# urw7rs/diffusion-models-made-easy

Hardware: AMD Instinct MI355X
Metric: denoising steps/sec + training images/sec, DDPM UNet CIFAR10 32×32 @1/2/4/8 GPU (higher is better)
Workload: dtype bf16

## Files before the change

### diffusion-models-made-easy_amd/csrc/conv_common.h

```cpp
#pragma once
#include <stdlib.h>

#include "common.h"

namespace dmme {

typedef float f32x16 __attribute__((ext_vector_type(16)));
typedef float f32x4 __attribute__((ext_vector_type(4)));
typedef __bf16 bf16x8 __attribute__((ext_vector_type(8)));
typedef f16 f16x8 __attribute__((ext_vector_type(8)));
template <typename T>
struct Vec8 {
    typedef T type __attribute__((ext_vector_type(8)));
};
template <typename T>
__device__ __forceinline__ void unpack8(const uint4& raw, float (&v)[8]) {
    const typename Vec8<T>::type x = __builtin_bit_cast(typename Vec8<T>::type, raw);
#pragma unroll
    for (int e = 0; e < 8; ++e) v[e] = (float)x[e];
}
template <typename T>
__device__ __forceinline__ uint4 pack8(const float (&v)[8]) {
    typename Vec8<T>::type x;
#pragma unroll
    for (int e = 0; e < 8; ++e) x[e] = (T)v[e];
    return __builtin_bit_cast(uint4, x);
}

constexpr int ROW_DATA = 128;
constexpr int ROW_PITCH = ROW_DATA + 16;

__device__ __forceinline__ int swz_off(int row, int chunk) { return row * ROW_DATA + ((chunk ^ ((row >> 1) & 7)) << 4); }

typedef __attribute__((address_space(3))) char lds_c;
__device__ __forceinline__ void glds16(const void* gsrc, unsigned lds_byte_addr) {
#if defined(__HIP_DEVICE_COMPILE__)
    __builtin_amdgcn_global_load_lds(gsrc, (lds_c*)(size_t)lds_byte_addr, 16, 0, 0);
#else
    (void)gsrc;
    (void)lds_byte_addr;
#endif
}
__device__ __forceinline__ void glds16_hidden(const void* gsrc, unsigned lds_byte_addr) {
#if defined(__HIP_DEVICE_COMPILE__)
    asm volatile("s_mov_b32 m0, %1\n\ts_nop 0\n\tglobal_load_lds_dwordx4 %0, off" ::"v"(gsrc), "s"(lds_byte_addr) : "m0");
#else
    (void)gsrc;
    (void)lds_byte_addr;
#endif
}
__device__ __forceinline__ void glds16_hidden_s(const void* sbase, unsigned lane_off, unsigned lds_byte_addr) {
#if defined(__HIP_DEVICE_COMPILE__)
    asm volatile("s_mov_b32 m0, %2\n\ts_nop 0\n\tglobal_load_lds_dwordx4 %0, %1" ::"v"(lane_off), "s"(sbase), "s"(lds_byte_addr) : "m0");
#else
    (void)sbase;
    (void)lane_off;
    (void)lds_byte_addr;
#endif
}
__device__ __forceinline__ void wait_vm_all() {
#if defined(__HIP_DEVICE_COMPILE__)
    asm volatile("s_waitcnt vmcnt(0)" ::: "memory");
#endif
}
__device__ __forceinline__ void wait_lgkm_all() {
#if defined(__HIP_DEVICE_COMPILE__)
    asm volatile("s_waitcnt lgkmcnt(0)" ::: "memory");
#endif
}
__device__ __forceinline__ void lds_barrier() {
#if defined(__HIP_DEVICE_COMPILE__)
    asm volatile("s_waitcnt lgkmcnt(0)" ::: "memory");
    __builtin_amdgcn_s_barrier();
    asm volatile("" ::: "memory");
#endif
}
template <int N>
__device__ __forceinline__ void wait_vm_keep() {
#if defined(__HIP_DEVICE_COMPILE__)
    asm volatile("s_waitcnt vmcnt(%0)" ::"n"(N) : "memory");
    asm volatile("s_waitcnt lgkmcnt(0)" ::: "memory");
#endif
}

template <typename T>
struct Frag;
template <>
struct Frag<float> {
    static constexpr int KC = 32;
    static constexpr int EPV = 4;
};
template <>
struct Frag<bf16> {
    static constexpr int KC = 64;
    static constexpr int EPV = 8;
};
template <>
struct Frag<f16> {
    static constexpr int KC = 64;
    static constexpr int EPV = 8;
};

__device__ __forceinline__ void mma_group(const uint4& a, const uint4& b, f32x16& acc, float*) {
    const f32x4 av = __builtin_bit_cast(f32x4, a), bv = __builtin_bit_cast(f32x4, b);
#pragma unroll
    for (int j = 0; j < 4; ++j) acc = __builtin_amdgcn_mfma_f32_32x32x2f32(av[j], bv[j], acc, 0, 0, 0);
}
__device__ __forceinline__ void mma_group(const uint4& a, const uint4& b, f32x16& acc, bf16*) {
    acc = __builtin_amdgcn_mfma_f32_32x32x16_bf16(__builtin_bit_cast(bf16x8, a), __builtin_bit_cast(bf16x8, b), acc, 0, 0, 0);
}
__device__ __forceinline__ void mma_group(const uint4& a, const uint4& b, f32x16& acc, f16*) {
    acc = __builtin_amdgcn_mfma_f32_32x32x16_f16(__builtin_bit_cast(f16x8, a), __builtin_bit_cast(f16x8, b), acc, 0, 0, 0);
}
template <typename T>
__device__ __forceinline__ void mma16(const uint4& a, const uint4& b, f32x16& acc) {
    mma_group(a, b, acc, (T*)nullptr);
}
template <typename T, typename A, typename B>
__device__ __forceinline__ f32x16 mma16v(const A& a, const B& b, f32x16 acc) {
    mma_group(__builtin_bit_cast(uint4, a), __builtin_bit_cast(uint4, b), acc, (T*)nullptr);
    return acc;
}

struct X3 {};
template <typename T, bool ACC3>
struct MmaTag {
    typedef T type;
};
template <>
struct MmaTag<float, true> {
    typedef X3 type;
};
typedef float f32x2 __attribute__((ext_vector_type(2)));
typedef __bf16 bf16x2 __attribute__((ext_vector_type(2)));
__device__ __forceinline__ float fma_plain(float a, float b, float c) {
    float d;
    asm("v_fma_f32 %0, %1, %2, %3" : "=v"(d) : "v"(a), "v"(b), "v"(c));
    return d;
}
__device__ __forceinline__ float mul_plain(float a, float b) {
    float d;
    asm("v_mul_f32 %0, %1, %2" : "=v"(d) : "v"(a), "v"(b));
    return d;
}
__device__ __forceinline__ float add_plain(float a, float b) {
    float d;
    asm("v_add_f32 %0, %1, %2" : "=v"(d) : "v"(a), "v"(b));
    return d;
}
__device__ __forceinline__ float sub_plain(float a, float b) {
    float d;
    asm("v_sub_f32 %0, %1, %2" : "=v"(d) : "v"(a), "v"(b));
    return d;
}
__device__ __forceinline__ float add1_plain(float a) {
    float d;
    asm("v_add_f32 %0, 1.0, %1" : "=v"(d) : "v"(a));
    return d;
}
__device__ __forceinline__ void pro_pair_plain(float x0, float x1, const f32x2& S, const f32x2& H, const f32x2& S2, const f32x2& H2, float& y0, float& y1) {
    float e0, e1;
    asm("v_fma_f32 %0, %4, %6, %8\n\t"
        "v_fma_f32 %2, %4, %10, %12\n\t"
        "v_fma_f32 %1, %5, %7, %9\n\t"
        "v_fma_f32 %3, %5, %11, %13\n\t"
        "v_exp_f32 %2, %2\n\t"
        "v_exp_f32 %3, %3\n\t"
        "v_add_f32 %2, 1.0, %2\n\t"
        "v_add_f32 %3, 1.0, %3\n\t"
        "v_rcp_f32 %2, %2\n\t"
        "v_rcp_f32 %3, %3\n\t"
        "v_mul_f32 %0, %0, %2\n\t"
        "v_mul_f32 %1, %1, %3"
        : "=&v"(y0), "=&v"(y1), "=&v"(e0), "=&v"(e1)
        : "v"(x0), "v"(x1), "v"(S[0]), "v"(S[1]), "v"(H[0]), "v"(H[1]), "v"(S2[0]), "v"(S2[1]), "v"(H2[0]), "v"(H2[1]));
}
typedef short s16x4 __attribute__((ext_vector_type(4)));
struct Split4 {
    uint2 hi, lo;
};
__device__ __forceinline__ unsigned pack_bf16(float a, float b) {
    const f32x2 v = {a, b};
    return __builtin_bit_cast(unsigned, __builtin_convertvector(v, bf16x2));
}
__device__ __forceinline__ Split4 split4(const uint4& v) {
    const f32x4 x = __builtin_bit_cast(f32x4, v);
    Split4 s;
    const unsigned h01 = pack_bf16(x[0], x[1]), h23 = pack_bf16(x[2], x[3]);
    s.hi = make_uint2(h01, h23);
    s.lo = make_uint2(pack_bf16(x[0] - __uint_as_float(h01 << 16), x[1] - __uint_as_float(h01 & 0xffff0000u)),
                      pack_bf16(x[2] - __uint_as_float(h23 << 16), x[3] - __uint_as_float(h23 & 0xffff0000u)));
    return s;
}
__device__ __forceinline__ void mma_x3(const Split4& a, const Split4& b, f32x16& acc) {
    const s16x4 ah = __builtin_bit_cast(s16x4, a.hi), al = __builtin_bit_cast(s16x4, a.lo);
// ... 746 lines not shown
```

### diffusion-models-made-easy_amd/csrc/conv_pipe.hip

```cpp
#include <stdio.h>

#include "conv_common.h"

namespace dmme {



template <typename T, int BM, int BN, int GT, int PIPE_UA, bool ACC3 = false>
__global__ void __launch_bounds__(256, GT == 9 ? 1 : 2) conv3x3_pipe_kernel(ConvArgs a, ConvTile g, int shTW, int shTH, int ksplit) {
    constexpr int KC = Frag<T>::KC, EPV = Frag<T>::EPV;
    constexpr int MI = BM / 64, NI = BN / 64;
    constexpr int UB = BN / 32;
    extern __shared__ __attribute__((aligned(16))) char lds[];
#define PIPE_STAMP(K) do { if (a.stamps && blockIdx.x < 2 && blockIdx.y == 0 && threadIdx.x == 0) a.stamps[blockIdx.x * 8 + (K)] = (long long)wall_clock64(); } while (0)
    PIPE_STAMP(0);
    char* ldsA = lds;
    char* ldsB = lds + (size_t)g.a_rows * ROW_DATA;
    constexpr bool DMAB_OK = sizeof(T) == 2 && GT == 3 && BN == 64;
    constexpr int B_BYTES = GT * BN * ROW_DATA;
    const bool dmab = DMAB_OK && a.dma_b;
    int cur = 0;
    float* gni_par = reinterpret_cast<float*>(ldsB + (size_t)B_BYTES * (dmab ? 2 : 1));

    const int tid = threadIdx.x, lane = tid & 63, wave = tid >> 6;
// ... 239 lines not shown
        }
        PIPE_STAMP(4);
        return;
    }
    if constexpr (BM == 64) {
        if (a.n_gno > 0) {
            const bool add_trow = a.tproj && a.nt != 1 && g.TN > 1;
            conv_epilogue_stage<T, BN, MI, NI>(a, acc, co0, wn0, r, h, wm0, n0, reinterpret_cast<float*>(lds), !add_trow);
            __syncthreads();
            conv_epilogue_store_direct<T, BN>(a, co0, n0, a.Hout * a.Wout, pix_of, reinterpret_cast<float*>(lds), add_trow);
            PIPE_STAMP(4);
            return;
        }
    }
    conv_epilogue<T, BM, BN, MI, NI>(a, acc, co0, wn0, r, h, wm0, n0, g.TN, pix_of, reinterpret_cast<float*>(lds), ty_blk * g.tiles_x + tx_blk);
    PIPE_STAMP(4);
#undef PIPE_STAMP
}

template <typename T>
__global__ void __launch_bounds__(256) conv_splitk_finish_kernel(ConvArgs a, int ksplit, int64_t total4) {
    const int C4 = a.Cout / 4, hw = a.Hout * a.Wout;
    const int64_t slice = (int64_t)a.N * hw * a.Cout;
    for (int64_t q = blockIdx.x * (int64_t)blockDim.x + threadIdx.x; q < total4; q += (int64_t)gridDim.x * blockDim.x) {
        const int64_t p = q / C4;
        const int c = (int)(q - p * C4) * 4;
        float4 v = *reinterpret_cast<const float4*>(a.splitk + p * a.Cout + c);
        for (int z = 1; z < ksplit; ++z) {
            const float4 u = *reinterpret_cast<const float4*>(a.splitk + z * slice + p * a.Cout + c);
            v.x += u.x; v.y += u.y; v.z += u.z; v.w += u.w;
        }
        float f[4] = {v.x, v.y, v.z, v.w};
        const int n = (int)(p / hw);
#pragma unroll
        for (int j = 0; j < 4; ++j) {
            float fold = a.bias ? a.bias[c + j] : 0.f;
            if (a.tproj) fold += a.tproj[(int64_t)(a.nt == 1 ? 0 : n) * a.tproj_ld + c + j];
            f[j] += fold;
            if (a.res1) f[j] += to_f(((const T*)a.res1)[p * a.Cout + c + j]);
            ((T*)a.dst)[p * a.Cout + c + j] = from_f<T>(f[j]);
        }
    }
}
static int pipe_ksplit(const ConvArgs& a, const ConvTile& g, int pick, int KC) {
    if (a.has_gni) return 1;
    const bool off = (debug_route("no_splitk") != 0);
    if (off || !a.splitk || pick != 3 || a.stride != 1 || a.gn_part || a.n_gno || a.out_silu || a.out_nchw || a.res2 || a.Cout % 4) return 1;
    const int64_t wgs = (int64_t)g.tiles_m * g.tiles_n;
    if (wgs > 128) return 1;
    int ks = (a.C1 + a.C2) / KC;
    const int room = (int)(256 / wgs);
    if (ks > room) ks = room;
    if (ks > 4) ks = 4;
    const int64_t out = (int64_t)a.N * a.Hout * a.Wout * a.Cout;
    while (ks > 1 && ks * out > a.splitk_cap) --ks;
    return ks < 1 ? 1 : ks;
}

#ifndef WS_CDMA
#define WS_CDMA 1
#endif
#ifndef WS_HYB
#define WS_HYB 0
#endif
#ifndef WS_SCHED2
#define WS_SCHED2 1
#endif
#ifndef WS_TP_UNROLL
#define WS_TP_UNROLL 9
#endif
template <typename T, int BN, int MI, int NI>
__device__ __forceinline__ void ws_stage16(const f32x16 (&acc)[MI][NI], T* row) {
    typedef T tx2 __attribute__((ext_vector_type(2)));
#pragma unroll
    for (int mi = 0; mi < MI; ++mi)
#pragma unroll
        for (int ni = 0; ni < NI; ++ni)
#pragma unroll
            for (int q = 0; q < 4; ++q) {
                const tx2 lo = {(T)acc[mi][ni][4 * q], (T)acc[mi][ni][4 * q + 1]}, hi = {(T)acc[mi][ni][4 * q + 2], (T)acc[mi][ni][4 * q + 3]};
                *reinterpret_cast<uint2*>(row + mi * 64 * (BN + kStage16Pad) + 32 * ni + 8 * q) = make_uint2(__builtin_bit_cast(unsigned, lo), __builtin_bit_cast(unsigned, hi));
            }
}
struct WsTile { int n0, oy0, ox0, co0, ts; };
__device__ __forceinline__ WsTile ws_tile_of(const ConvTile& g, int shTW, int shTH, int kt, int bn) {
    const int t = (int)blockIdx.x + kt * (int)gridDim.x;
    const int tile_n = t % g.tiles_n, tile_m = t / g.tiles_n;
    const int tiles_img = g.tiles_x * g.tiles_y;
    WsTile r;
    const int sp = tile_m % tiles_img;
    r.n0 = tile_m / tiles_img;
    r.oy0 = (sp / g.tiles_x) << shTH;
    r.ox0 = (sp % g.tiles_x) << shTW;
    r.co0 = tile_n * bn;
    r.ts = sp;
    return r;
}

__host__ __device__ inline int ws2_stage_pad(int a_bytes) { return a_bytes + 2 * 128 * ROW_DATA >= 64 * 1024 ? 0 : 64 * 1024 - 2 * 128 * ROW_DATA - a_bytes; }

__device__ __forceinline__ void ws_fill_par_gni(const ConvArgs& a, int n, bool writer, float* par, int Cin, int tid, int nthr) {
    for (int c = tid; c < Cin; c += nthr) {
        float sc, sh;
        const float dmk = a.dmask ? a.dmask[n * Cin + c] : 1.f;
        gn_in_scale_shift(a, n, c, Cin, writer, sc, sh);
        par[c] = sc * dmk;
        par[Cin + c] = sh * dmk;
        par[2 * Cin + c] = a.pro_silu ? -1.4426950408889634f * sc : 0.f;
        par[3 * Cin + c] = a.pro_silu ? -1.4426950408889634f * sh : -126.f;
    }
}

template <typename T, int SPLIT>
struct WsSplit {
    typedef T ts;
};
template <typename T>
struct WsSplit<T, 1> {
    typedef float ts;
};
template <typename T>
struct WsSplit<T, 2> {
    typedef float ts;
};
template <int PIPE_UA, typename T = bf16, int BM = 256, int SPLIT = 0, bool RSEG = false, bool E16 = false>
__global__ void __launch_bounds__(512, 1) conv3x3_ws2_kernel(ConvArgs a, ConvTile g, int shTW, int shTH, int ntiles) {
    constexpr int KC = 64, EPV = 8, BN = 128, MI = BM / 64, NI = 2, UB = BN / 32;
    constexpr bool CDMA = WS_CDMA != 0;
    constexpr bool SCHED2 = WS_SCHED2 != 0 && CDMA && SPLIT == 0;
    static_assert(!(SCHED2 && WS_HYB != 0), "the hybrid tap ownership counts the halo loads of the two-unit schedule");
    static_assert(!E16 || (SPLIT == 0 && BM == 256 && sizeof(T) == 2), "16-bit staging: 16-bit tensors, 256-pixel tiles");
    static_assert(!RSEG || (SPLIT == 0 && sizeof(T) == 2), "residual segment: 16-bit tensors");
    constexpr int KCR = SPLIT ? 32 : KC;
    constexpr int EPR = SPLIT ? 4 : EPV;
    typedef typename WsSplit<T, SPLIT>::ts TS;
    static_assert(SPLIT == 0 || (BM == 256 && dtype_of<T>::value == DMME_F16), "split passes: fp16 hi / lo on the 256-pixel tile");
    constexpr int R_BYTES = BN * ROW_DATA;
    constexpr int A_PITCH = ROW_DATA + 16;
    static_assert((BM == 256 && PIPE_UA == 11) || (BM == 128 && PIPE_UA == 7), "unit schedules below: 11 units over 9 stages, or 7 units over the first 7");
    typedef unsigned u32x4 __attribute__((ext_vector_type(4)));
    extern __shared__ __attribute__((aligned(16))) char lds[];
    const int a_bytes = g.a_rows * A_PITCH;
    const int Cin = a.C1 + a.C2;
    const int offA1 = a_bytes + 3 * R_BYTES, offR = a_bytes;
    float* par_base = reinterpret_cast<float*>(lds + 2 * a_bytes + 3 * R_BYTES + ws2_stage_pad(a_bytes));
    float* fold_base = par_base + 2 * 4 * Cin;
#define WS_FILL_FOLD(KT)                                                                              \
    if constexpr (E16) {                                                                              \
        if (tid < BN) {                                                                               \
            const TileXY ff_ = WS_TILE(KT);                                                           \
            const int co_ = ff_.co0 + tid;                                                            \
            float f_ = 0.f;                                                                           \
            if (co_ < a.Cout) {                                                                       \
                f_ = a.bias ? a.bias[co_] : 0.f;                                                      \
                if (a.r_bias) f_ += a.r_bias[co_];                                                    \
                if (a.tproj) f_ += a.tproj[(a.nt == 1 ? 0 : ff_.n0) * a.tproj_ld + co_];              \
            }                                                                                         \
            fold_base[((KT) & 1) * BN + tid] = f_;                                                    \
        }                                                                                             \
    }
#define WS_BUFA(p) (lds + (((p) & 1) ? offA1 : 0))
#define WS_RING(slot) (lds + offR + (slot) * R_BYTES)
#define WS_PAR(kt) (par_base + ((kt) & 1) * 4 * Cin)
#define WS_TILE(kt) ws_tile_of(g, shTW, shTH, (kt), BN)
    typedef WsTile TileXY;
    const int tid = threadIdx.x, lane = tid & 63, wave = tid >> 6;
    const bool producer = wave >= 4;
    const int nchunks = Cin / KCR;
    const int CinW = SPLIT ? 2 * Cin : Cin;
    const int Cres = RSEG ? a.r_C1 + a.r_C2 : 0;
    const int HS = Cres / 32;
    constexpr int RSL = 5;
    const int RT = HS + ((RSEG && (HS - 1) % RSL < 2) ? 1 : 0);
#define WS_RSA(k) ((k) < 2 ? lds + (k) * (BM * 64) : (k) == 2 ? lds + offR + 2 * R_BYTES : lds + offA1 + ((k) - 3) * (BM * 64))
#define WS_RSW(k) ((k) < 4 ? lds + offR + (k) * 8192 : lds + offA1 + 2 * (BM * 64))
    const int K = (ntiles - (int)blockIdx.x + (int)gridDim.x - 1) / (int)gridDim.x;
    const bool has_pro = a.scale || a.pro_silu || a.dmask;
#define WS_FILL_PAR_N(KT, NTHR)                                           \
    {                                                                     \
        float* par = WS_PAR(KT);                                          \
        const TileXY ft_ = WS_TILE(KT);                                   \
        if (a.has_gni) {                                                  \
            ws_fill_par_gni(a, ft_.n0, ft_.ts == 0 && ft_.co0 == 0, par, Cin, tid, NTHR); \
        } else {                                                          \
            const int pn0 = ft_.n0;                                       \
            for (int c = tid; c < Cin; c += (NTHR)) {                     \
                const int so = pn0 * Cin + c;                             \
                const float sc_ = a.scale ? a.scale[so] : 1.f, sh_ = a.scale ? a.shift[so] : 0.f, dm_ = a.dmask ? a.dmask[so] : 1.f; \
                par[c] = sc_ * dm_;                                       \
                par[Cin + c] = sh_ * dm_;                                 \
                par[2 * Cin + c] = a.pro_silu ? -1.4426950408889634f * sc_ : 0.f;    \
                par[3 * Cin + c] = a.pro_silu ? -1.4426950408889634f * sh_ : -126.f; \
            }                                                             \
        }                                                                 \
    }
#define WS_FILL_PAR(KT) WS_FILL_PAR_N(KT, 512)
    const int mTW = (1 << shTW) - 1, mTH = (1 << shTH) - 1;
    float gn_carry[2] = {0.f, 0.f};
    const bool estamp = tid == 0 && blockIdx.x == 0;
    int e_i = 0;
#define WS_ESTAMP() { if (estamp && a.stamps && e_i < 24) a.stamps[64 + e_i++] = (long long)clock64(); }
#define WS2_PASS(TT, P, STAGE_STMT)                                                                                                \
    {                                                                                                                              \
        constexpr int p = (P);                                                                                                     \
        auto pix_of = [&](int m) -> int {                                                                                          \
            const int mm = m + 128 * p;                                                                                            \
            const int tx = mm & mTW, ty = (mm >> shTW) & mTH;                                                                      \
            return ((TT).n0 * a.Hout + (TT).oy0 + ty) * a.Wout + (TT).ox0 + tx;                                                    \
        };                                                                                                                         \
        uint4 rpre[128 * (BN / (16 / (int)sizeof(TS))) / 512];                                                                     \
        if constexpr (!E16) conv_epilogue_res_prefetch<TS, 128, BN, 512>(a, (TT).co0, pix_of, rpre);  \
        WS_ESTAMP()                                                                                                                \
        STAGE_STMT                                                                                                                 \
        WS_ESTAMP()                                                                                                                \
        lds_barrier();                                                                                                             \
// ... 369 lines not shown
                        }                                                                                               \
                        __builtin_amdgcn_sched_barrier(0);                                                              \
                        const int hmax = j + 4 < HS - 1 ? j + 4 : HS - 1;     \
                        const int ahead = hmax - (j + 1);                    \
                        if (fin) wait_vm_keep<UB + PIPE_UA>();                                                          \
                        else if (ahead >= 3) wait_vm_keep<3 * RD>();                                                    \
                        else if (ahead == 2) wait_vm_keep<2 * RD>();                                                    \
                        else if (ahead == 1) wait_vm_keep<RD>();                                                        \
                        else wait_vm_keep<0>();                                                                         \
                        __builtin_amdgcn_s_barrier();                                                                   \
                    }                                                                                                   \
                }                                                                                                       \
                if constexpr (E16) { WS2_EPILOGUE16(tcur, kt, ;) } else { WS2_EPILOGUE(tcur, kt, ;, ;) }                         \
                                       \
                        \
                cc = 0;                                                                                                 \
                ++kt;                                                                                                   \
                tcur = tnext;                                                                                           \
                tnext = WS_TILE(kt + 1 < K ? kt + 1 : kt);                                                              \
            }                                                                                                           \
        }                                                                                                               \
    }
        const int GCH = K * nchunks;
        for (int ch = 0; ch < GCH; ++ch) {
            WS_PSTAGE(0) WS_PSTAGE(1) WS_PSTAGE(2) WS_PSTAGE(3) WS_PSTAGE(4) WS_PSTAGE(5) WS_PSTAGE(6) WS_PSTAGE(7) WS_PSTAGE(8)
        }
#ifdef WS_PSTAMPS
        if (a.stamps && ptid == 0 && blockIdx.x == 0)
            for (int i = 0; i < p_i; ++i) a.stamps[128 + i] = pst_lds[i];
#endif
#undef WS_PSTAGE
#undef WS_RD
#undef WS_RX
#undef WS_L
#undef WS_PST
#undef WS_PSTT
#undef WS_A_UNIT
#undef WS_A_MATH
#undef WS_A_WRITE
#undef WS_A_ARRIVED
        return;
    }

    WS_FILL_PAR(0)
    WS_FILL_FOLD(0)
    __syncthreads();
    if (K > 1) WS_FILL_PAR_N(1, 256)
    __builtin_amdgcn_s_setprio(3);
    const int wrow = wave >> 1, wn0 = (wave & 1) * 64;
    const int r = lane & 31, h = lane >> 5;
    int a_row[MI];
#pragma unroll
    for (int mi = 0; mi < MI; ++mi) {
        const int m = (2 * mi + wrow) * 32 + r;
        const int tx = m & mTW, ty = (m >> shTW) & mTH;
        a_row[mi] = (ty * g.HWd + tx) * A_PITCH + h * 16;
    }
    int b_off[NI][4];
#pragma unroll
    for (int ni = 0; ni < NI; ++ni) {
        const int row = wn0 + ni * 32 + r;
#pragma unroll
        for (int kg = 0; kg < 4; ++kg) b_off[ni][kg] = row * ROW_DATA + (((kg * 2 + h) ^ ((row >> 1) & 7)) << 4);
    }
    unsigned cb_vo[UB];
#pragma unroll
    for (int k4 = 0; k4 < UB; ++k4) {
        const int urow_ = wave * 8 + (lane >> 3);
        cb_vo[k4] = (unsigned)(((urow_ + 32 * k4) * 9 * CinW + ((lane & 7) ^ ((urow_ >> 1) & 7)) * EPV) * 2);
    }
    auto cdma = [&](int slot, int co0, int c, int t) __attribute__((always_inline)) {
        const char* ub = (const char*)a.w + ((size_t)co0 * 9 * CinW + (size_t)t * CinW + (size_t)c * KC) * 2;
        const unsigned lbase = (unsigned)(size_t)(lds_c*)WS_RING(slot) + (unsigned)(wave * 8 * ROW_DATA);
#pragma unroll
        for (int k4 = 0; k4 < UB; ++k4)
            glds16_hidden_s(ub, cb_vo[k4], (unsigned)__builtin_amdgcn_readfirstlane((int)(lbase + (unsigned)(32 * k4 * ROW_DATA))));
    };
    int stamp_i = 0;
    const bool stamping = a.stamps && tid == 0 && blockIdx.x == 0;
#define WS_STAMP() { if (stamping && stamp_i < 64) a.stamps[stamp_i++] = (long long)clock64(); }
    WS_STAMP()
    __syncthreads();
    WS_STAMP()
    int cg = 0;
    for (int kt = 0; kt < K; ++kt) {
        const TileXY t = WS_TILE(kt);
        f32x16 acc[MI][NI];
        if constexpr (E16) {
            const float* fb = fold_base + (kt & 1) * BN + wn0 + 4 * h;
#pragma unroll
            for (int ni = 0; ni < NI; ++ni)
#pragma unroll
                for (int q = 0; q < 4; ++q) {
                    const f32x4 f4 = *reinterpret_cast<const f32x4*>(fb + 32 * ni + 8 * q);
#pragma unroll
                    for (int mi = 0; mi < MI; ++mi)
#pragma unroll
                        for (int k = 0; k < 4; ++k) acc[mi][ni][4 * q + k] = f4[k];
                }
        } else {
#pragma unroll
        for (int mi = 0; mi < MI; ++mi)
#pragma unroll
            for (int ni = 0; ni < NI; ++ni)
#pragma unroll
                for (int j = 0; j < 16; ++j) acc[mi][ni][j] = 0.f;
        }
#if defined(WS_X_NO_FRAGS)
#define WS_FRAGS(SET, KG)                                                                                                         \
    {                                                                                                                             \
        _Pragma("unroll") for (int mi = 0; mi < MI; ++mi) { u32x4 t_; asm volatile("" : "=v"(t_)); af[SET][mi] = __builtin_bit_cast(uint4, t_); }   \
        _Pragma("unroll") for (int ni = 0; ni < NI; ++ni) { u32x4 t_; asm volatile("" : "=v"(t_)); bfr[SET][ni] = __builtin_bit_cast(uint4, t_); }  \
        __builtin_amdgcn_sched_barrier(0);                                                                                        \
    }
#else
#define WS_FRAGS(SET, KG)                                                                                                         \
    {                                                                                                                             \
        _Pragma("unroll") for (int mi = 0; mi < MI; ++mi) af[SET][mi] = *reinterpret_cast<const uint4*>(pa[mi] + (KG) * 32);      \
        _Pragma("unroll") for (int ni = 0; ni < NI; ++ni) bfr[SET][ni] = *reinterpret_cast<const uint4*>(ldsR + b_off[ni][KG]);   \
        __builtin_amdgcn_sched_barrier(0);                                                                                        \
    }
#endif
#if defined(WS_X_NO_MFMA)
#define WS_MMAS(SET)                                                                                  \
    {                                                                                                 \
        _Pragma("unroll") for (int mi = 0; mi < MI; ++mi) asm volatile("" ::"v"(__builtin_bit_cast(u32x4, af[SET][mi])));   \
        _Pragma("unroll") for (int ni = 0; ni < NI; ++ni) asm volatile("" ::"v"(__builtin_bit_cast(u32x4, bfr[SET][ni])));  \
        __builtin_amdgcn_sched_barrier(0);                                                            \
    }
#else
#define WS_MMAS(SET)                                                                                  \
    {                                                                                                 \
        _Pragma("unroll") for (int mi = 0; mi < MI; ++mi)                                             \
            _Pragma("unroll") for (int ni = 0; ni < NI; ++ni) {                                       \
                if constexpr (E16) mma_group(bfr[SET][ni], af[SET][mi], acc[mi][ni], (T*)nullptr);    \
                else mma_group(af[SET][mi], bfr[SET][ni], acc[mi][ni], (T*)nullptr);                  \
            }                                                                                         \
        __builtin_amdgcn_sched_barrier(0);                                                            \
    }
#endif
#define WS_FA(SET, KG) { _Pragma("unroll") for (int mi = 0; mi < MI; ++mi) af[SET][mi] = *reinterpret_cast<const uint4*>(pa[mi] + (KG) * 32); }
#define WS_FB(SET, KG) { _Pragma("unroll") for (int ni = 0; ni < NI; ++ni) bfr[SET][ni] = *reinterpret_cast<const uint4*>(ldsR + b_off[ni][KG]); }
#define WS_SB() __builtin_amdgcn_sched_barrier(0);
#define WS_MM(SA, SB_)                                                                                \
    {                                                                                                 \
        _Pragma("unroll") for (int mi = 0; mi < MI; ++mi)                                             \
            _Pragma("unroll") for (int ni = 0; ni < NI; ++ni) mma_group(af[SA][mi], bfr[SB_][ni], acc[mi][ni], (T*)nullptr); \
        __builtin_amdgcn_sched_barrier(0);                                                            \
    }
        const TileXY tn = WS_TILE(kt + 1 < K ? kt + 1 : kt);
        const bool three = !a.mix2;
        for (int c = 0; c < nchunks; ++c, ++cg) {
            const char* ldsA = WS_BUFA(cg);
            const bool last_c = c + 1 == nchunks;
#pragma unroll WS_TP_UNROLL
            for (int tp = 0; tp < 9; ++tp) {
                const char* ldsR = WS_RING(tp % 3);
                const int tap_b = ((tp / 3) * g.HWd + (tp % 3)) * A_PITCH;
                const char* pa[MI];
#pragma unroll
                for (int mi = 0; mi < MI; ++mi) pa[mi] = ldsA + a_row[mi] + tap_b;
                uint4 af[2][MI], bfr[2][NI];
                bool sent = false;
#define WS_CDMA_ISSUE()                                                                                               \
    if constexpr (CDMA) {                                                                                             \
        if (tp == 0 && c == 0 && kt > 0) cdma(1, t.co0, 0, 1);                                                        \
        if (tp <= 6) { if (WS_HYB == 0 || tp == 0 || tp == 6) { cdma((tp + 2) % 3, t.co0, c, tp + 2); sent = true; } } \
        else if (RSEG && last_c) { }                                                                                  \
        else if (tp == 7) { if (!(last_c && kt + 1 == K)) { cdma(0, last_c ? tn.co0 : t.co0, last_c ? 0 : c + 1, 0); sent = true; } } \
        else if (!last_c) { cdma(1, t.co0, c + 1, 1); sent = true; }                                                  \
        __builtin_amdgcn_sched_barrier(0);                                                                            \
    }
                if constexpr (SPLIT != 0) {
                    WS_FA(0, 0) WS_FB(0, 0) WS_FB(1, 2) WS_SB()
                    WS_CDMA_ISSUE()
                    WS_MM(0, 0)
                    WS_FA(1, 2) WS_SB()
                    if (three) { WS_MM(0, 1) }
                    WS_FA(0, 1) WS_FB(1, 1) WS_SB()
                    WS_MM(1, 0)
                    WS_FB(0, 3) WS_FA(1, 3) WS_SB()
                    WS_MM(0, 1)
                    if (three) { WS_MM(0, 0) }
                    WS_MM(1, 1)
                } else {
                    WS_FRAGS(0, 0) WS_FRAGS(1, 1) WS_CDMA_ISSUE() WS_MMAS(0) WS_FRAGS(0, 2) WS_MMAS(1) WS_FRAGS(1, 3) WS_MMAS(0) WS_MMAS(1)
                }
#undef WS_CDMA_ISSUE
                WS_STAMP()
                if constexpr (CDMA) {
                    if (sent) wait_vm_keep<UB>();
                    else wait_vm_keep<0>();
                }
                __syncthreads();
                WS_STAMP()
            }
        }
        if constexpr (RSEG) {
            const int rsw = (r >> 2) & 3;
            const int rA = (wrow * 32 + r) * 64, rB = (wn0 + r) * 64;
            const int pk0 = (h ^ rsw) << 4, pk1 = ((2 + h) ^ rsw) << 4;
            int slot = 0;
            for (int j = 0; j < HS; ++j) {
                const char* sa = WS_RSA(slot) + rA;
                const char* sw = WS_RSW(slot) + rB;
                slot = slot == RSL - 1 ? 0 : slot + 1;
                uint4 af[2][MI], bfr[2][NI];
#pragma unroll
                for (int mi = 0; mi < MI; ++mi) af[0][mi] = *reinterpret_cast<const uint4*>(sa + mi * 4096 + pk0);
#pragma unroll
                for (int ni = 0; ni < NI; ++ni) bfr[0][ni] = *reinterpret_cast<const uint4*>(sw + ni * 2048 + pk0);
                __builtin_amdgcn_sched_barrier(0);
#pragma unroll
                for (int mi = 0; mi < MI; ++mi) af[1][mi] = *reinterpret_cast<const uint4*>(sa + mi * 4096 + pk1);
#pragma unroll
                for (int ni = 0; ni < NI; ++ni) bfr[1][ni] = *reinterpret_cast<const uint4*>(sw + ni * 2048 + pk1);
                __builtin_amdgcn_sched_barrier(0);
                WS_MMAS(0) WS_MMAS(1)
                WS_STAMP()
                __syncthreads();
                WS_STAMP()
            }
            for (int j = HS; j < RT; ++j) __syncthreads();
        }
#undef WS_FA
#undef WS_FB
#undef WS_SB
#undef WS_MM
#undef WS_FRAGS
#undef WS_MMAS
        if constexpr (E16) {
            WS2_EPILOGUE16(t, kt, (ws_stage16<T, BN, MI, NI>(acc, st16 + (wrow * 32 + r) * (BN + kStage16Pad) + wn0 + 4 * h));)
        } else {
        WS2_EPILOGUE(t, kt, (conv_epilogue_stage<T, BN, 2, NI, 64>(a, reinterpret_cast<f32x16(&)[2][NI]>(acc[0]), t.co0, wn0, r, h, wrow * 32, t.n0, stage));,
                     (conv_epilogue_stage<T, BN, 2, NI, 64>(a, reinterpret_cast<f32x16(&)[2][NI]>(acc[2]), t.co0, wn0, r, h, wrow * 32, t.n0, stage));)
        }
        WS_STAMP()
    }
#undef WS_STAMP
#undef WS2_EPILOGUE
#undef WS2_EPILOGUE16
#undef WS_FILL_FOLD
#undef WS2_PASS
#undef WS_FILL_PAR
#undef WS_FILL_PAR_N
#undef WS_ESTAMP
#undef WS_BUFA
#undef WS_RING
#undef WS_RSA
#undef WS_RSW
#undef WS_PAR
#undef WS_TILE
}

static size_t ws2_lds(const ConvArgs& a, const ConvTile& g) {
    const size_t a_bytes = (size_t)g.a_rows * (ROW_DATA + 16);
    size_t extra = 0;
#ifdef WS_PSTAMPS
    extra = 4096;
#endif
    return 2 * a_bytes + 3 * (size_t)128 * ROW_DATA + (size_t)ws2_stage_pad((int)a_bytes) + (size_t)2 * 4 * (a.C1 + a.C2) * 4 + 1024  + extra;
}

static int ws_pick(const ConvArgs& a, ConvTile& g) {
    constexpr int ws_min_tiles = 256;
    const int Cin = a.C1 + a.C2, nch = Cin / 64;
    if (a.taps != 9 || a.stride != 1 || Cin % 64 || a.C1 % 64 || nch < 2 || nch % 2 || Cin > 512 || a.out_silu || a.out_nchw || a.in_nchw || a.Cout % 128) return 0;
    ConvTile t;
    if (make_tile(a, 256, 128, t) && t.TN == 1 && t.a_rows <= 352 && ws2_lds(a, t) <= 160 * 1024 && (size_t)t.a_rows * ROW_DATA + 2 * 128 * ROW_DATA >= 64 * 1024 &&
        t.tiles_m * t.tiles_n >= ws_min_tiles) {
        g = t;
        return 3;
    }
    ConvTile u;
    if (!debug_route("no_ws128") && make_tile(a, 128, 128, u) && u.TN == 1 && u.a_rows <= 224 && ws2_lds(a, u) <= 160 * 1024 && u.tiles_m * u.tiles_n >= ws_min_tiles) {
        g = u;
        return 4;
    }
    return 0;
}

static bool ws2s_pick(const ConvArgs& a, ConvTile& g) {
    const int Cin = a.C1 + a.C2;
    if ((a.mix != 1 && a.mix != 2) || a.taps != 9 || a.stride != 1 || a.up == 2 || Cin % 64 || a.C1 % 32 || Cin < 64 || Cin > 512 || a.out_silu || a.out_nchw || a.in_nchw ||
        a.Cout % 128 || a.res2 || a.n_gno || (a.tproj && a.nt != 1 && a.nt != a.N))
        return false;
    if ((int64_t)a.Cout * 9 * 2 * Cin >= (1ll << 30) || (int64_t)a.N * a.Hin * a.Win * Cin >= (1ll << 29)) return false;
    ConvTile t;
    if (!make_tile(a, 256, 128, t) || t.TN != 1 || t.a_rows > 352 || ws2_lds(a, t) > 160 * 1024 || (size_t)t.a_rows * ROW_DATA + 2 * 128 * ROW_DATA < 64 * 1024) return false;
    g = t;
    return true;
}
static const int kPipeCand[5][3] = {{128, 128, 3}, {128, 64, 3}, {64, 64, 3}, {64, 64, 9}, {64, 64, 3}};
static const int kPipeUA[5] = {8, 8, 8, 11, 10};
static size_t pipe_lds(const ConvTile& g, int BN, int GT) { return (size_t)g.a_rows * ROW_DATA + (size_t)GT * BN * ROW_DATA; }
static bool pipe_dma_ok(int dtype, const ConvTile& g, int BN, int GT) {
    const bool off = (debug_route("no_pipe_dma") != 0);
    return !off && is16(dtype) && GT == 3 && BN == 64 && pipe_lds(g, BN, GT) + (size_t)GT * BN * ROW_DATA <= 80 * 1024;
}

static int ilog2(int v) {
    int s = 0;
    while ((1 << s) < v) ++s;
    return s;
}

static bool pipe_fits(const ConvArgs& a, int i, ConvTile& t) {
    if (!make_tile(a, kPipeCand[i][0], kPipeCand[i][1], t)) return false;
    if (t.a_rows * 8 > 256 * kPipeUA[i]) return false;
    if (pipe_lds(t, kPipeCand[i][1], kPipeCand[i][2]) > (kPipeCand[i][2] == 9 ? 128 : 80) * 1024) return false;
    if (a.Cout <= 64 && kPipeCand[i][1] > 64) return false;
    return true;
}

static int pipe_pick(const ConvArgs& a, ConvTile& g) {
    int pick = -1;
    if (a.stride == 1)
        for (int i = 0; i < 3; ++i) {
            ConvTile t;
            if (!pipe_fits(a, i, t)) continue;
            pick = i;
            g = t;
// ... 27 lines not shown
    ConvTile gw{};
    return ws_pick(a, gw) != 0;
}

bool conv_pipe_supported(int dtype, const ConvArgs& a) {
    if (a.mix) {
        ConvTile gs{};
        return dtype == DMME_F16 && a.taps == 9 && ws2s_pick(a, gs);
    }
    if (!conv_mfma_supported(dtype, a)) return false;
    if (a.taps != 9 || (a.stride != 1 && a.stride != 2)) return false;
    if ((int64_t)a.Cout * 9 * (a.C1 + a.C2) >= (1ll << 31)) return false;
    if ((int64_t)a.N * a.Hin * a.Win >= (1ll << 31)) return false;
    ConvTile g;
    return pipe_pick(a, g) >= 0;
}

template <typename K>
static int set_lds_limit(K kernel, size_t bytes) {
    DMME_CHECK_HIP(hipFuncSetAttribute(reinterpret_cast<const void*>(kernel), hipFuncAttributeMaxDynamicSharedMemorySize, (int)bytes));
    return DMME_OK;
}

static int launch_ws2_split(const ConvArgs& a, hipStream_t s) {
    ConvTile gw{};
    DMME_REQUIRE(ws2s_pick(a, gw), DMME_ERR_UNSUPPORTED, "conv3x3 (split fp16 passes): unsupported shape");
    static bool attr = false;
    if (!attr) {
        int rc0 = set_lds_limit(conv3x3_ws2_kernel<11, f16, 256, 1>, 160 * 1024);
        if (rc0 == DMME_OK) rc0 = set_lds_limit(conv3x3_ws2_kernel<11, f16, 256, 2>, 160 * 1024);
        if (rc0 != DMME_OK) return rc0;
        attr = true;
    }
    const int ntiles = gw.tiles_m * gw.tiles_n;
    const dim3 wgrid((unsigned)(ntiles < 256 ? ntiles : 256));
    if (a.mix == 2)
        hipLaunchKernelGGL((conv3x3_ws2_kernel<11, f16, 256, 2>), wgrid, dim3(512), ws2_lds(a, gw), s, a, gw, ilog2(gw.TW), ilog2(gw.TH), ntiles);
    else
        hipLaunchKernelGGL((conv3x3_ws2_kernel<11, f16, 256, 1>), wgrid, dim3(512), ws2_lds(a, gw), s, a, gw, ilog2(gw.TW), ilog2(gw.TH), ntiles);
    DMME_CHECK_LAUNCH();
    return DMME_OK;
}

static bool kw_takes(int dtype, const ConvArgs& a, int pick, ConvTile& gk, int* ni, int* ring, int* bm) {
    constexpr int all = 0;
    if (pick != 3 && pick != 2) return false;
    if (!conv_kw_pick(dtype, a, gk, ni, ring, bm)) return false;
    return pick == 3 || all || *bm == 128;
}
static int kw_ksplit(const ConvArgs&, const ConvTile&) { return 1; }
template <typename T>
static int launch_kw_t(const ConvArgs& a, const ConvTile& gk, int ni, int ring, int bm, hipStream_t s) {
    const int ksplit = kw_ksplit(a, gk);
    const int rc = launch_conv_kw(dtype_of<T>::value, a, gk, ni, ring, bm, ksplit, s);
    if (rc != DMME_OK) return rc;
    if (ksplit > 1) {
        const int64_t total4 = (int64_t)a.N * a.Hout * a.Wout * (a.Cout / 4);
        hipLaunchKernelGGL(conv_splitk_finish_kernel<T>, dim3((unsigned)((total4 + 255) / 256)), dim3(256), 0, s, a, ksplit, total4);
        DMME_CHECK_LAUNCH();
    }
    return DMME_OK;
}

template <typename T, bool ACC3 = false>
static int launch_pipe_t(const ConvArgs& a, hipStream_t s) {
    ConvTile g{};
    const int pick = pipe_pick(a, g);
    DMME_REQUIRE(pick >= 0, DMME_ERR_UNSUPPORTED, "conv_pipe: no tile fits");
    const int ksplit = pipe_ksplit(a, g, pick, Frag<T>::KC);
    const dim3 grid((unsigned)(g.tiles_m * g.tiles_n), (unsigned)ksplit);
    if constexpr (sizeof(T) == 2) {
        const bool ws_off = getenv("DMME_NO_WS") != nullptr;
        ConvTile gw{};
        const int ws = ws_off ? 0 : ws_pick(a, gw);
        if (ws) {
            static bool ws_attr = false;
            if (!ws_attr) {
                int rc0 = set_lds_limit(conv3x3_ws2_kernel<11, T, 256>, 160 * 1024);
                if (rc0 == DMME_OK) rc0 = set_lds_limit(conv3x3_ws2_kernel<7, T, 128>, 160 * 1024);
                if (rc0 == DMME_OK) rc0 = set_lds_limit(conv3x3_ws2_kernel<11, T, 256, 0, true>, 160 * 1024);
                if (rc0 == DMME_OK) rc0 = set_lds_limit(conv3x3_ws2_kernel<7, T, 128, 0, true>, 160 * 1024);
                if (rc0 == DMME_OK) rc0 = set_lds_limit(conv3x3_ws2_kernel<11, T, 256, 0, false, true>, 160 * 1024);
                if (rc0 == DMME_OK) rc0 = set_lds_limit(conv3x3_ws2_kernel<11, T, 256, 0, true, true>, 160 * 1024);
                if (rc0 != DMME_OK) return rc0;
                ws_attr = true;
            }
            const int ntiles = gw.tiles_m * gw.tiles_n;
            const dim3 wgrid((unsigned)(ntiles < 256 ? ntiles : 256));
            const bool e16 = !a.res1 && !a.res2 && !debug_route("no_ws_e16");
            if (a.r_w) {
                DMME_REQUIRE(rseg_shape_ok(a), DMME_ERR_UNSUPPORTED, "conv3x3 with a residual segment: raw channel counts outside the wave-specialised kernel's domain");
                if (ws == 4)
                    hipLaunchKernelGGL((conv3x3_ws2_kernel<7, T, 128, 0, true>), wgrid, dim3(512), ws2_lds(a, gw), s, a, gw, ilog2(gw.TW), ilog2(gw.TH), ntiles);
                else if (e16)
                    hipLaunchKernelGGL((conv3x3_ws2_kernel<11, T, 256, 0, true, true>), wgrid, dim3(512), ws2_lds(a, gw), s, a, gw, ilog2(gw.TW), ilog2(gw.TH), ntiles);
                else
                    hipLaunchKernelGGL((conv3x3_ws2_kernel<11, T, 256, 0, true>), wgrid, dim3(512), ws2_lds(a, gw), s, a, gw, ilog2(gw.TW), ilog2(gw.TH), ntiles);
            } else if (ws == 4)
                hipLaunchKernelGGL((conv3x3_ws2_kernel<7, T, 128>), wgrid, dim3(512), ws2_lds(a, gw), s, a, gw, ilog2(gw.TW), ilog2(gw.TH), ntiles);
            else if (e16)
                hipLaunchKernelGGL((conv3x3_ws2_kernel<11, T, 256, 0, false, true>), wgrid, dim3(512), ws2_lds(a, gw), s, a, gw, ilog2(gw.TW), ilog2(gw.TH), ntiles);
            else
                hipLaunchKernelGGL((conv3x3_ws2_kernel<11, T, 256>), wgrid, dim3(512), ws2_lds(a, gw), s, a, gw, ilog2(gw.TW), ilog2(gw.TH), ntiles);
            DMME_CHECK_LAUNCH();
            return DMME_OK;
        }
    }
    DMME_REQUIRE(!a.r_w, DMME_ERR_UNSUPPORTED, "conv3x3 with a residual segment: only the wave-specialised kernel takes it");
    if constexpr (sizeof(T) == 2) {
        ConvTile gk{};
        int kni = 0, kring = 0, kbm = 0;
        if (kw_takes(dtype_of<T>::value, a, pick, gk, &kni, &kring, &kbm)) return launch_kw_t<T>(a, gk, kni, kring, kbm, s);
    }
    size_t lds = pipe_lds(g, kPipeCand[pick][1], kPipeCand[pick][2]);
    ConvArgs ad = a;
    ad.dma_b = (sizeof(T) == 2 && !ACC3 && pipe_dma_ok(dtype_of<T>::value, g, kPipeCand[pick][1], kPipeCand[pick][2])) ? 1 : 0;
    if (ad.dma_b) lds += (size_t)kPipeCand[pick][2] * kPipeCand[pick][1] * ROW_DATA;
    if (a.has_gni) lds += (size_t)2 * (a.C1 + a.C2) * 4;
    if (a.n_gno && lds < (size_t)kDirectLds) lds = kDirectLds;
    const int shTW = ilog2(g.TW), shTH = ilog2(g.TH);
    static bool attr_done[5] = {false, false, false, false, false};
    int rc = DMME_OK;
#define DMME_PIPE_CASE(IDX, BM_, BN_, GT_, UA_, LIM)                                                                          \
    case IDX:                                                                                                                 \
        if (!attr_done[IDX]) {                                                                                                \
            rc = set_lds_limit(conv3x3_pipe_kernel<T, BM_, BN_, GT_, UA_, ACC3>, (LIM) * 1024);                               \
            attr_done[IDX] = rc == DMME_OK;                                                                                   \
        }                                                                                                                     \
        if (rc == DMME_OK) hipLaunchKernelGGL((conv3x3_pipe_kernel<T, BM_, BN_, GT_, UA_, ACC3>), grid, dim3(256), lds, s, ad, g, shTW, shTH, ksplit); \
        break;
    switch (pick) {
        DMME_PIPE_CASE(0, 128, 128, 3, 8, 80)
        DMME_PIPE_CASE(1, 128, 64, 3, 8, 80)
        DMME_PIPE_CASE(2, 64, 64, 3, 8, 80)
        DMME_PIPE_CASE(3, 64, 64, 9, 11, 128)
        DMME_PIPE_CASE(4, 64, 64, 3, 10, 80)
    }
#undef DMME_PIPE_CASE
    if (rc != DMME_OK) return rc;
    DMME_CHECK_LAUNCH();
    if (ksplit > 1) {
        const int64_t total4 = (int64_t)a.N * a.Hout * a.Wout * (a.Cout / 4);
        hipLaunchKernelGGL(conv_splitk_finish_kernel<T>, dim3((unsigned)((total4 + 255) / 256)), dim3(256), 0, s, a, ksplit, total4);
        DMME_CHECK_LAUNCH();
    }
    return DMME_OK;
}

int launch_conv_pipe(int dtype, const ConvArgs& a, hipStream_t s) {
    DMME_REQUIRE(conv_pipe_supported(dtype, a), DMME_ERR_UNSUPPORTED, "conv_pipe: unsupported shape");
    if (a.mix) return launch_ws2_split(a, s);
    if (dtype == DMME_BF16) return launch_pipe_t<bf16>(a, s);
    if (dtype == DMME_F16) return launch_pipe_t<f16>(a, s);
    return a.x3 ? launch_pipe_t<float, true>(a, s) : launch_pipe_t<float>(a, s);
}

bool conv_gn_in_query(int dtype, const ConvArgs& a) {
    if (getenv("DMME_NO_GN_IN") || !is16(dtype)) return false;
    if (conv_out_thin_supported(dtype, a)) return true;
    if (a.mix) return conv_pipe_supported(dtype, a);
    if (a.taps == 1) return conv1x1_as_supported(dtype, a) || conv1x1_pipe_gn_in_ok(dtype, a);
    if (!conv_pipe_supported(dtype, a)) return false;
    ConvTile gw{};
    if (!getenv("DMME_NO_WS") && ws_pick(a, gw)) return true;
    ConvTile g{}, gk{};
    const int pick = pipe_pick(a, g);
    int kni = 0, kring = 0, kbm = 0;
    if (pick < 0) return false;
    if (!debug_route("no_gn_in_kw") && kw_takes(dtype, a, pick, gk, &kni, &kring, &kbm)) return gk.TN == 1 && kw_ksplit(a, gk) == 1;
    if (kw_takes(dtype, a, pick, gk, &kni, &kring, &kbm)) return false;
    if (debug_route("no_gn_in_pipe") || g.TN != 1) return false;
    ConvArgs b = a;
    b.has_gni = 1;
    b.splitk = nullptr;
    size_t lds = pipe_lds(g, kPipeCand[pick][1], kPipeCand[pick][2]);
    if (pipe_dma_ok(dtype, g, kPipeCand[pick][1], kPipeCand[pick][2])) lds += (size_t)kPipeCand[pick][2] * kPipeCand[pick][1] * ROW_DATA;
    lds += (size_t)2 * (a.C1 + a.C2) * 4;
    return lds <= (size_t)(kPipeCand[pick][2] == 9 ? 128 : 80) * 1024;
}

bool conv_gn_direct_query(int dtype, const ConvArgs& a, const int* cg, int n) {
    const bool off = getenv("DMME_NO_GN_DIRECT") != nullptr;
// ... 116 lines not shown
```

Measured before the change: 459.9.

## Add 16x16x32 MFMA consumer path to wave-specialised conv3x3 kernel

Adds an M16 variant of the wave-specialised 3x3 conv kernel that uses 16x16x32 bf16/f16 MFMA instructions with a new fragment layout, register accumulators of 8x4 f32x4, and its own staging routine. It also prefetches the next tap's pixel fragments across the tap boundary and replaces the full vm+lgkm wait plus syncthreads with a barrier that waits only on vector memory. The goal is better MFMA issue density and less stall at tap boundaries. The path is on by default for the non-residual E16 route. It adds new LDS access patterns and a new synchronisation scheme that could affect correctness or bank conflicts.

```diff
diff --git a/diffusion-models-made-easy_amd/csrc/conv_common.h b/diffusion-models-made-easy_amd/csrc/conv_common.h
--- a/diffusion-models-made-easy_amd/csrc/conv_common.h
+++ b/diffusion-models-made-easy_amd/csrc/conv_common.h
@@ -71,6 +71,14 @@
 __device__ __forceinline__ void lds_barrier() {
 #if defined(__HIP_DEVICE_COMPILE__)
     asm volatile("s_waitcnt lgkmcnt(0)" ::: "memory");
+    __builtin_amdgcn_s_barrier();
+    asm volatile("" ::: "memory");
+#endif
+}
+template <int N>
+__device__ __forceinline__ void vm_barrier_keep_lds() {
+#if defined(__HIP_DEVICE_COMPILE__)
+    asm volatile("s_waitcnt vmcnt(%0)" ::"n"(N) : "memory");
     __builtin_amdgcn_s_barrier();
     asm volatile("" ::: "memory");
 #endif
@@ -111,6 +119,12 @@
 }
 __device__ __forceinline__ void mma_group(const uint4& a, const uint4& b, f32x16& acc, f16*) {
     acc = __builtin_amdgcn_mfma_f32_32x32x16_f16(__builtin_bit_cast(f16x8, a), __builtin_bit_cast(f16x8, b), acc, 0, 0, 0);
+}
+__device__ __forceinline__ f32x4 mma_16x16(const uint4& a, const uint4& b, f32x4 acc, bf16*) {
+    return __builtin_amdgcn_mfma_f32_16x16x32_bf16(__builtin_bit_cast(bf16x8, a), __builtin_bit_cast(bf16x8, b), acc, 0, 0, 0);
+}
+__device__ __forceinline__ f32x4 mma_16x16(const uint4& a, const uint4& b, f32x4 acc, f16*) {
+    return __builtin_amdgcn_mfma_f32_16x16x32_f16(__builtin_bit_cast(f16x8, a), __builtin_bit_cast(f16x8, b), acc, 0, 0, 0);
 }
 template <typename T>
 __device__ __forceinline__ void mma16(const uint4& a, const uint4& b, f32x16& acc) {
diff --git a/diffusion-models-made-easy_amd/csrc/conv_pipe.hip b/diffusion-models-made-easy_amd/csrc/conv_pipe.hip
--- a/diffusion-models-made-easy_amd/csrc/conv_pipe.hip
+++ b/diffusion-models-made-easy_amd/csrc/conv_pipe.hip
@@ -345,6 +345,17 @@
                 *reinterpret_cast<uint2*>(row + mi * 64 * (BN + kStage16Pad) + 32 * ni + 8 * q) = make_uint2(__builtin_bit_cast(unsigned, lo), __builtin_bit_cast(unsigned, hi));
             }
 }
+template <typename T, int BN>
+__device__ __forceinline__ void ws_stage16_m16(const f32x4 (&acc)[8][4], T* row) {
+    typedef T tx2 __attribute__((ext_vector_type(2)));
+#pragma unroll
+    for (int b = 0; b < 8; ++b)
+#pragma unroll
+        for (int nb = 0; nb < 4; ++nb) {
+            const tx2 lo = {(T)acc[b][nb][0], (T)acc[b][nb][1]}, hi = {(T)acc[b][nb][2], (T)acc[b][nb][3]};
+            *reinterpret_cast<uint2*>(row + ((b >> 1) * 64 + (b & 1)) * (BN + kStage16Pad) + 16 * nb) = make_uint2(__builtin_bit_cast(unsigned, lo), __builtin_bit_cast(unsigned, hi));
+        }
+}
 struct WsTile { int n0, oy0, ox0, co0, ts; };
 __device__ __forceinline__ WsTile ws_tile_of(const ConvTile& g, int shTW, int shTH, int kt, int bn) {
     const int t = (int)blockIdx.x + kt * (int)gridDim.x;
@@ -386,7 +397,10 @@
 struct WsSplit<T, 2> {
     typedef float ts;
 };
-template <int PIPE_UA, typename T = bf16, int BM = 256, int SPLIT = 0, bool RSEG = false, bool E16 = false>
+#ifndef WS_M16_PRE
+#define WS_M16_PRE 1
+#endif
+template <int PIPE_UA, typename T = bf16, int BM = 256, int SPLIT = 0, bool RSEG = false, bool E16 = false, bool M16 = false>
 __global__ void __launch_bounds__(512, 1) conv3x3_ws2_kernel(ConvArgs a, ConvTile g, int shTW, int shTH, int ntiles) {
     constexpr int KC = 64, EPV = 8, BN = 128, MI = BM / 64, NI = 2, UB = BN / 32;
     constexpr bool CDMA = WS_CDMA != 0;
@@ -394,6 +408,7 @@
     static_assert(!(SCHED2 && WS_HYB != 0), "the hybrid tap ownership counts the halo loads of the two-unit schedule");
     static_assert(!E16 || (SPLIT == 0 && BM == 256 && sizeof(T) == 2), "16-bit staging: 16-bit tensors, 256-pixel tiles");
     static_assert(!RSEG || (SPLIT == 0 && sizeof(T) == 2), "residual segment: 16-bit tensors");
+    static_assert(!M16 || E16, "16x16x32 consumers: the transposed, 16-bit staged form");
     constexpr int KCR = SPLIT ? 32 : KC;
     constexpr int EPR = SPLIT ? 4 : EPV;
     typedef typename WsSplit<T, SPLIT>::ts TS;
@@ -929,9 +944,107 @@
     WS_STAMP()
     __syncthreads();
     WS_STAMP()
+#define WS_CDMA_ISSUE()                                                                                               \
+    if constexpr (CDMA) {                                                                                             \
+        if (tp == 0 && c == 0 && kt > 0) cdma(1, t.co0, 0, 1);                                                        \
+        if (tp <= 6) { if (WS_HYB == 0 || tp == 0 || tp == 6) { cdma((tp + 2) % 3, t.co0, c, tp + 2); sent = true; } } \
+        else if (RSEG && last_c) { }                                                                                  \
+        else if (tp == 7) { if (!(last_c && kt + 1 == K)) { cdma(0, last_c ? tn.co0 : t.co0, last_c ? 0 : c + 1, 0); sent = true; } } \
+        else if (!last_c) { cdma(1, t.co0, c + 1, 1); sent = true; }                                                  \
+        __builtin_amdgcn_sched_barrier(0);                                                                            \
+    }
+    const int j16 = lane & 15, q16 = lane >> 4;
+    int a_row16 = 0, b_off16 = 0, a_mi16 = 0;
+    if constexpr (M16) {
+        const int m = wrow * 32 + 2 * j16;
+        a_row16 = (((m >> shTW) & mTH) * g.HWd + (m & mTW)) * A_PITCH + q16 * 16;
+        a_mi16 = (64 >> shTW) * g.HWd * A_PITCH;
+        b_off16 = (wn0 + j16) * ROW_DATA + ((q16 ^ ((j16 >> 1) & 7)) << 4);
+    }
     int cg = 0;
     for (int kt = 0; kt < K; ++kt) {
         const TileXY t = WS_TILE(kt);
+        if constexpr (M16) {
+            f32x4 acc4[8][4];
+            {
+                const float* fb = fold_base + (kt & 1) * BN + wn0 + 4 * q16;
+#pragma unroll
+                for (int nb = 0; nb < 4; ++nb) {
+                    const f32x4 f4 = *reinterpret_cast<const f32x4*>(fb + 16 * nb);
+#pragma unroll
+                    for (int b = 0; b < 8; ++b) acc4[b][nb] = f4;
+                }
+            }
+            const TileXY tn = WS_TILE(kt + 1 < K ? kt + 1 : kt);
+            uint4 px[3], fw[2][4];
+#define WS16_PX(TP, I) px[(16 * (TP) + (I)) % 3] = *reinterpret_cast<const uint4*>(ldsA + a_row16 + (((I) & 7) >> 1) * a_mi16 + (((TP) / 3) * g.HWd + (TP) % 3 + ((I) & 1)) * A_PITCH + ((I) >> 3) * 64)
+#define WS16_FW(KS, NB) fw[KS][NB] = *reinterpret_cast<const uint4*>(ldsR + (b_off16 ^ ((KS) * 64)) + (NB) * 16 * ROW_DATA)
+            for (int c = 0; c < nchunks; ++c, ++cg) {
+                const char* ldsA = WS_BUFA(cg);
+                const bool last_c = c + 1 == nchunks;
+#pragma unroll
+                for (int tp = 0; tp < 9; ++tp) {
+                    const char* ldsR = WS_RING(tp % 3);
+                    const bool own = tp == 0 || WS_M16_PRE == 0;
+                    bool sent = false;
+                    WS16_FW(0, 0);
+                    if (own) WS16_PX(tp, 0);
+                    WS16_FW(0, 1); WS16_FW(0, 2); WS16_FW(0, 3);
+                    if (own) WS16_PX(tp, 1);
+                    __builtin_amdgcn_sched_barrier(0);
+                    WS_CDMA_ISSUE()
+#pragma unroll
+                    for (int i = 0; i < 16; ++i) {
+#pragma unroll
+                        for (int nb = 0; nb < 4; ++nb) acc4[i & 7][nb] = mma_16x16(fw[i >> 3][nb], px[(16 * tp + i) % 3], acc4[i & 7][nb], (T*)nullptr);
+                        if (i + 2 < 16) WS16_PX(tp, i + 2);
+                        else if (WS_M16_PRE != 0 && tp < 8) WS16_PX(tp + 1, i + 2 - 16);
+                        if (i >= 1 && i <= 4) WS16_FW(1, i - 1);
+                        __builtin_amdgcn_sched_barrier(0);
+                    }
+                    WS_STAMP()
+                    if (WS_M16_PRE != 0 && tp < 8) {
+                        if (sent) vm_barrier_keep_lds<UB>();
+                        else vm_barrier_keep_lds<0>();
+                    } else {
+                        if (sent) wait_vm_keep<UB>();
+                        else wait_vm_keep<0>();
+                        __syncthreads();
+                    }
+                    WS_STAMP()
+                }
+            }
+#undef WS16_PX
+#undef WS16_FW
+            if constexpr (RSEG) {
+                const int pkA = (q16 ^ ((j16 >> 1) & 3)) << 4, pkB = (q16 ^ ((j16 >> 2) & 3)) << 4;
+                const int rA = (wrow * 32 + 2 * j16) * 64 + pkA, rB = (wn0 + j16) * 64 + pkB;
+                int slot = 0;
+                for (int j = 0; j < HS; ++j) {
+                    const char* sa = WS_RSA(slot) + rA;
+                    const char* sw = WS_RSW(slot) + rB;
+                    slot = slot == RSL - 1 ? 0 : slot + 1;
+                    uint4 pxr[8], fwr[4];
+#pragma unroll
+                    for (int nb = 0; nb < 4; ++nb) fwr[nb] = *reinterpret_cast<const uint4*>(sw + nb * 1024);
+#pragma unroll
+                    for (int b = 0; b < 8; ++b) pxr[b] = *reinterpret_cast<const uint4*>(sa + (b >> 1) * 4096 + (b & 1) * 64);
+                    __builtin_amdgcn_sched_barrier(0);
+#pragma unroll
+                    for (int b = 0; b < 8; ++b)
+#pragma unroll
+                        for (int nb = 0; nb < 4; ++nb) acc4[b][nb] = mma_16x16(fwr[nb], pxr[b], acc4[b][nb], (T*)nullptr);
+                    __builtin_amdgcn_sched_barrier(0);
+                    WS_STAMP()
+                    __syncthreads();
+                    WS_STAMP()
+                }
+                for (int j = HS; j < RT; ++j) __syncthreads();
+            }
+            WS2_EPILOGUE16(t, kt, (ws_stage16_m16<T, BN>(acc4, st16 + (wrow * 32 + 2 * j16) * (BN + kStage16Pad) + wn0 + 4 * q16));)
+            WS_STAMP()
+            continue;
+        }
         f32x16 acc[MI][NI];
         if constexpr (E16) {
             const float* fb = fold_base + (kt & 1) * BN + wn0 + 4 * h;
@@ -1009,15 +1122,6 @@
                 for (int mi = 0; mi < MI; ++mi) pa[mi] = ldsA + a_row[mi] + tap_b;
                 uint4 af[2][MI], bfr[2][NI];
                 bool sent = false;
-#define WS_CDMA_ISSUE()                                                                                               \
-    if constexpr (CDMA) {                                                                                             \
-        if (tp == 0 && c == 0 && kt > 0) cdma(1, t.co0, 0, 1);                                                        \
-        if (tp <= 6) { if (WS_HYB == 0 || tp == 0 || tp == 6) { cdma((tp + 2) % 3, t.co0, c, tp + 2); sent = true; } } \
-        else if (RSEG && last_c) { }                                                                                  \
-        else if (tp == 7) { if (!(last_c && kt + 1 == K)) { cdma(0, last_c ? tn.co0 : t.co0, last_c ? 0 : c + 1, 0); sent = true; } } \
-        else if (!last_c) { cdma(1, t.co0, c + 1, 1); sent = true; }                                                  \
-        __builtin_amdgcn_sched_barrier(0);                                                                            \
-    }
                 if constexpr (SPLIT != 0) {
                     WS_FA(0, 0) WS_FB(0, 0) WS_FB(1, 2) WS_SB()
                     WS_CDMA_ISSUE()
@@ -1033,7 +1137,6 @@
                 } else {
                     WS_FRAGS(0, 0) WS_FRAGS(1, 1) WS_CDMA_ISSUE() WS_MMAS(0) WS_FRAGS(0, 2) WS_MMAS(1) WS_FRAGS(1, 3) WS_MMAS(0) WS_MMAS(1)
                 }
-#undef WS_CDMA_ISSUE
                 WS_STAMP()
                 if constexpr (CDMA) {
                     if (sent) wait_vm_keep<UB>();
@@ -1085,6 +1188,7 @@
         WS_STAMP()
     }
 #undef WS_STAMP
+#undef WS_CDMA_ISSUE
 #undef WS2_EPILOGUE
 #undef WS2_EPILOGUE16
 #undef WS_FILL_FOLD
@@ -1278,22 +1382,29 @@
                 if (rc0 == DMME_OK) rc0 = set_lds_limit(conv3x3_ws2_kernel<7, T, 128, 0, true>, 160 * 1024);
                 if (rc0 == DMME_OK) rc0 = set_lds_limit(conv3x3_ws2_kernel<11, T, 256, 0, false, true>, 160 * 1024);
                 if (rc0 == DMME_OK) rc0 = set_lds_limit(conv3x3_ws2_kernel<11, T, 256, 0, true, true>, 160 * 1024);
+                if (rc0 == DMME_OK) rc0 = set_lds_limit(conv3x3_ws2_kernel<11, T, 256, 0, false, true, true>, 160 * 1024);
+                if (rc0 == DMME_OK) rc0 = set_lds_limit(conv3x3_ws2_kernel<11, T, 256, 0, true, true, true>, 160 * 1024);
                 if (rc0 != DMME_OK) return rc0;
                 ws_attr = true;
             }
             const int ntiles = gw.tiles_m * gw.tiles_n;
             const dim3 wgrid((unsigned)(ntiles < 256 ? ntiles : 256));
             const bool e16 = !a.res1 && !a.res2 && !debug_route("no_ws_e16");
+            const bool m16 = e16 && !debug_route("ws_mfma32") && (!a.r_w || debug_route("ws_mfma16_res"));
             if (a.r_w) {
                 DMME_REQUIRE(rseg_shape_ok(a), DMME_ERR_UNSUPPORTED, "conv3x3 with a residual segment: raw channel counts outside the wave-specialised kernel's domain");
                 if (ws == 4)
                     hipLaunchKernelGGL((conv3x3_ws2_kernel<7, T, 128, 0, true>), wgrid, dim3(512), ws2_lds(a, gw), s, a, gw, ilog2(gw.TW), ilog2(gw.TH), ntiles);
+                else if (m16)
+                    hipLaunchKernelGGL((conv3x3_ws2_kernel<11, T, 256, 0, true, true, true>), wgrid, dim3(512), ws2_lds(a, gw), s, a, gw, ilog2(gw.TW), ilog2(gw.TH), ntiles);
                 else if (e16)
                     hipLaunchKernelGGL((conv3x3_ws2_kernel<11, T, 256, 0, true, true>), wgrid, dim3(512), ws2_lds(a, gw), s, a, gw, ilog2(gw.TW), ilog2(gw.TH), ntiles);
                 else
                     hipLaunchKernelGGL((conv3x3_ws2_kernel<11, T, 256, 0, true>), wgrid, dim3(512), ws2_lds(a, gw), s, a, gw, ilog2(gw.TW), ilog2(gw.TH), ntiles);
             } else if (ws == 4)
                 hipLaunchKernelGGL((conv3x3_ws2_kernel<7, T, 128>), wgrid, dim3(512), ws2_lds(a, gw), s, a, gw, ilog2(gw.TW), ilog2(gw.TH), ntiles);
+            else if (m16)
+                hipLaunchKernelGGL((conv3x3_ws2_kernel<11, T, 256, 0, false, true, true>), wgrid, dim3(512), ws2_lds(a, gw), s, a, gw, ilog2(gw.TW), ilog2(gw.TH), ntiles);
             else if (e16)
                 hipLaunchKernelGGL((conv3x3_ws2_kernel<11, T, 256, 0, false, true>), wgrid, dim3(512), ws2_lds(a, gw), s, a, gw, ilog2(gw.TW), ilog2(gw.TH), ntiles);
             else
```

Result: no change. 460.5 (median of 6 runs) (+0.1%).
